# XiaoWang-Github/ORBIT-2

Measured on AMD Instinct MI355X. Metric: climate-grid samples/sec/node (fwd+bwd), interm_1b ERA5 1.4°→0.25°, 1/2/4/8 GPUs, higher is better.
Workload: dtype bf16

## Files before the change

orbit-2_amd/csrc/image.hip:

```cpp
#include "common.h"
#include "../../include/orbit2_hip.h"

namespace {

inline int grid_for(int64_t n, int per_block) {
  int64_t g = (n + per_block - 1) / per_block;
  if (g < 1) g = 1;
  if (g > 8192) g = 8192;
  return (int)g;
}

template <bool BWD, bool T_FP32 = false>
__global__ __launch_bounds__(256) void unpatchify_kernel(bf16_t* __restrict__ t, float* __restrict__ img, int B, int C,
                                                         int Hh, int Wh, int p) {
  const int64_t per = (int64_t)C * Hh * Wh;
  const int64_t n = (int64_t)B * per;
  const int wf = Wh / p;
  for (int64_t e = (int64_t)blockIdx.x * 256 + threadIdx.x; e < n; e += (int64_t)gridDim.x * 256) {
    const int b = (int)(e / per);
    int64_t r = e - (int64_t)b * per;
    if (!BWD) {
      const int c = (int)(r / ((int64_t)Hh * Wh));
      r -= (int64_t)c * Hh * Wh;
      const int y = (int)(r / Wh), x = (int)(r - (int64_t)y * Wh);
      const int hh = y / p, pp = y - hh * p, ww = x / p, qq = x - ww * p;
      const int64_t ti = ((((int64_t)hh * wf + ww) * p + pp) * p + qq) * C + c;
      img[e] = T_FP32 ? reinterpret_cast<const float*>(t)[(int64_t)b * per + ti] : bf2f(t[(int64_t)b * per + ti]);
    } else {
      const int c = (int)(r % C);
      int64_t q = r / C;
      const int qq = (int)(q % p); q /= p;
      const int pp = (int)(q % p); q /= p;
      const int ww = (int)(q % wf);
      const int hh = (int)(q / wf);
      t[e] = f2bf(img[(int64_t)b * per + ((int64_t)c * Hh + (hh * p + pp)) * Wh + (ww * p + qq)]);
    }
  }
}

constexpr int CONV_MAXCIN = 8;
constexpr int COB = 16;
__global__ __launch_bounds__(256) void conv3x3_fwd_kernel(const float* __restrict__ in, const int* __restrict__ cidx,
                                                          int in_ctotal, const float* __restrict__ wgt,
                                                          const float* __restrict__ bias, float* __restrict__ out,
                                                          float* __restrict__ pre, const float* __restrict__ addend,
                                                          int Ha, int Wa, int B, int Cin, int Cout, int H, int W,
                                                          int mode, int r) {
  __shared__ float sw[COB * CONV_MAXCIN * 9 + COB];
  const int co0 = blockIdx.y * COB;
  const int nco = (Cout - co0) < COB ? (Cout - co0) : COB;
  for (int e = threadIdx.x; e < nco * Cin * 9; e += 256) sw[e] = wgt[(size_t)co0 * Cin * 9 + e];
  for (int e = threadIdx.x; e < nco; e += 256) sw[COB * CONV_MAXCIN * 9 + e] = bias[co0 + e];
  __syncthreads();
  const int64_t npix = (int64_t)B * H * W;
  for (int64_t px = (int64_t)blockIdx.x * 256 + threadIdx.x; px < npix; px += (int64_t)gridDim.x * 256) {
    const int b = (int)(px / ((int64_t)H * W));
    const int rem = (int)(px - (int64_t)b * H * W);
    const int y = rem / W, x = rem - y * W;
    float nb[CONV_MAXCIN][9];
#pragma unroll
    for (int ci = 0; ci < CONV_MAXCIN; ++ci) {
      if (ci < Cin) {
        const int cs = cidx ? cidx[ci] : ci;
        const float* pl = in + ((size_t)b * in_ctotal + cs) * H * W;
#pragma unroll
        for (int k = 0; k < 9; ++k) {
          const int yy = y + k / 3 - 1, xx = x + k % 3 - 1;
          nb[ci][k] = (yy >= 0 && yy < H && xx >= 0 && xx < W) ? pl[(size_t)yy * W + xx] : 0.f;
        }
      }
    }
    for (int co = 0; co < nco; ++co) {
      float acc = sw[COB * CONV_MAXCIN * 9 + co];
#pragma unroll
      for (int ci = 0; ci < CONV_MAXCIN; ++ci) {
        if (ci < Cin) {
#pragma unroll
          for (int k = 0; k < 9; ++k) acc = fmaf(sw[(co * Cin + ci) * 9 + k], nb[ci][k], acc);
        }
      }
      const int cg = co0 + co;
      if (mode == 0) {
        if (addend) acc += addend[(((size_t)b * Cout + cg) * Ha + y) * Wa + x];
        out[(((size_t)b * Cout + cg) * H + y) * W + x] = acc;
      } else {
        pre[(((size_t)b * Cout + cg) * H + y) * W + x] = acc;
        const int rr = r * r;
        const int oc = cg / rr, sub = cg - oc * rr;
        out[(((size_t)b * (Cout / rr) + oc) * (H * r) + (y * r + sub / r)) * (size_t)(W * r) + (x * r + sub % r)] =
            gelu_f(acc);
      }
    }
  }
}

__device__ __forceinline__ float conv_dpre(const float* __restrict__ dout, const float* __restrict__ pre, int b,
                                           int co, int y, int x, int Cout, int H, int W, int mode, int r) {
  if (mode == 0) return dout[(((size_t)b * Cout + co) * H + y) * W + x];
  const int rr = r * r;
  const int oc = co / rr, sub = co - oc * rr;
  const float d =
      dout[(((size_t)b * (Cout / rr) + oc) * (H * r) + (y * r + sub / r)) * (size_t)(W * r) + (x * r + sub % r)];
  return d * dgelu_f(pre[(((size_t)b * Cout + co) * H + y) * W + x]);
}

__global__ __launch_bounds__(256) void conv3x3_bwd_data_kernel(const float* __restrict__ dout,
                                                               const float* __restrict__ pre,
                                                               const float* __restrict__ wgt, float* __restrict__ din,
                                                               int B, int Cin, int Cout, int H, int W, int mode,
                                                               int r) {
  const int64_t n = (int64_t)B * Cin * H * W;
  for (int64_t e = (int64_t)blockIdx.x * 256 + threadIdx.x; e < n; e += (int64_t)gridDim.x * 256) {
    int64_t q = e;
    const int x = (int)(q % W); q /= W;
    const int y = (int)(q % H); q /= H;
    const int ci = (int)(q % Cin);
    const int b = (int)(q / Cin);
    float acc = 0.f;
    for (int co = 0; co < Cout; ++co) {
#pragma unroll
      for (int k = 0; k < 9; ++k) {
        const int yy = y + 1 - k / 3, xx = x + 1 - k % 3;
        if (yy >= 0 && yy < H && xx >= 0 && xx < W)
          acc = fmaf(conv_dpre(dout, pre, b, co, yy, xx, Cout, H, W, mode, r), wgt[((size_t)co * Cin + ci) * 9 + k],
                     acc);
      }
    }
    din[e] = acc;
  }
}

constexpr int TW = 16, TH = 16;
__global__ __launch_bounds__(256) void conv3x3_bwd_weight_kernel(const float* __restrict__ dout,
                                                                 const float* __restrict__ pre,
                                                                 const float* __restrict__ in,
                                                                 const int* __restrict__ cidx, int in_ctotal,
                                                                 float* __restrict__ ws,
                                                                 int B, int Cin, int Cout, int H, int W, int mode,
                                                                 int r) {
  float* dw = ws + ((size_t)blockIdx.y * gridDim.x + blockIdx.x) * ((size_t)Cout * Cin * 9 + Cout);
  float* dbias = dw + (size_t)Cout * Cin * 9;
  __shared__ float sd[COB][TH][TW];
  __shared__ float si[CONV_MAXCIN][TH + 2][TW + 2];
  const int tiles_x = (W + TW - 1) / TW;
  const int ty0 = (blockIdx.x / tiles_x) * TH, tx0 = (blockIdx.x % tiles_x) * TW;
  const int b = blockIdx.y;
  for (int e = threadIdx.x; e < Cin * (TH + 2) * (TW + 2); e += 256) {
    const int ci = e / ((TH + 2) * (TW + 2));
    const int rem = e - ci * (TH + 2) * (TW + 2);
    const int yy = ty0 + rem / (TW + 2) - 1, xx = tx0 + rem % (TW + 2) - 1;
    const int cs = cidx ? cidx[ci] : ci;
    si[ci][rem / (TW + 2)][rem % (TW + 2)] =
        (yy >= 0 && yy < H && xx >= 0 && xx < W) ? in[(((size_t)b * in_ctotal + cs) * H + yy) * W + xx] : 0.f;
  }
  for (int co0 = 0; co0 < Cout; co0 += COB) {
    const int nco = (Cout - co0) < COB ? (Cout - co0) : COB;
    __syncthreads();
    for (int e = threadIdx.x; e < nco * TH * TW; e += 256) {
      const int co = e / (TH * TW);
      const int rem = e - co * TH * TW;
      const int y = ty0 + rem / TW, x = tx0 + rem % TW;
      sd[co][rem / TW][rem % TW] =
          (y < H && x < W) ? conv_dpre(dout, pre, b, co0 + co, y, x, Cout, H, W, mode, r) : 0.f;
    }
    __syncthreads();
    for (int e = threadIdx.x; e < nco * Cin * 9; e += 256) {
      const int co = e / (Cin * 9);
      const int rem = e - co * Cin * 9;
      const int ci = rem / 9, k = rem - ci * 9;
      const int ky = k / 3, kx = k - ky * 3;
      float s = 0.f;
      for (int y = 0; y < TH; ++y)
#pragma unroll
        for (int x = 0; x < TW; ++x) s = fmaf(sd[co][y][x], si[ci][y + ky][x + kx], s);
      dw[((size_t)(co0 + co) * Cin + ci) * 9 + k] = s;
    }
    for (int co = threadIdx.x; co < nco; co += 256) {
      float s = 0.f;
      for (int y = 0; y < TH; ++y)
        for (int x = 0; x < TW; ++x) s += sd[co][y][x];
      dbias[co0 + co] = s;
    }
  }
}

__global__ __launch_bounds__(256) void clamp_channel_kernel(float* __restrict__ img, const float* __restrict__ ref,
                                                            float* __restrict__ dimg, int B, int C, int HW,
                                                            int chan) {
  const int64_t n = (int64_t)B * HW;
  for (int64_t e = (int64_t)blockIdx.x * 256 + threadIdx.x; e < n; e += (int64_t)gridDim.x * 256) {
    const int b = (int)(e / HW);
    const size_t off = ((size_t)b * C + chan) * HW + (e - (int64_t)b * HW);
    if (dimg) { if (!(ref[off] > 0.f)) dimg[off] = 0.f; }
    else img[off] = fmaxf(img[off], 0.f);
  }
}

__device__ __forceinline__ float sgn(float v) { return (v > 0.f) ? 1.f : ((v < 0.f) ? -1.f : 0.f); }

__global__ __launch_bounds__(256) void loss_fwd_kernel(const float* __restrict__ pred, const float* __restrict__ tgt,
                                                       int Ht, int Wt, const float* __restrict__ latw,
                                                       const float* __restrict__ chanw, float* __restrict__ part,
                                                       float* __restrict__ part2, int C, int H, int W, int kind) {
  const int plane = blockIdx.y;
  const int c = plane % C, b = plane / C;
  const float* p = pred + (size_t)plane * H * W;
  const float* t = tgt + ((size_t)b * C + c) * Ht * Wt;
  const float cw = chanw ? chanw[c] : 1.f;
  float s = 0.f, s2 = 0.f;
  for (int e = blockIdx.x * 256 + threadIdx.x; e < H * W; e += gridDim.x * 256) {
    const int i = e / W, j = e - i * W;
    const float pv = p[e];
    const float tv0 = t[(size_t)i * Wt + j];
    const float d = pv - tv0;
    float err = d * d;
// ... 109 lines not shown
  const int64_t n = (int64_t)B * C * h * s * w * s;
  hipLaunchKernelGGL(unpatchify_kernel<false>, dim3(grid_for(n, 256)), dim3(256), 0, (hipStream_t)stream, (bf16_t*)t,
                     img, B, C, h * s, w * s, p);
  O2_CHECK_LAUNCH();
  return O2_OK;
}
extern "C" int orbit2_unpatchify_fwd_f32(const float* t, float* img, int B, int C, int h, int w, int p, int s,
                                         void* stream) {
  if (!t || !img || B <= 0 || C <= 0 || p <= 0 || s <= 0 || (h * s) % p || (w * s) % p) return O2_ERR_ARG;
  const int64_t n = (int64_t)B * C * h * s * w * s;
  hipLaunchKernelGGL((unpatchify_kernel<false, true>), dim3(grid_for(n, 256)), dim3(256), 0, (hipStream_t)stream,
                     (bf16_t*)t, img, B, C, h * s, w * s, p);
  O2_CHECK_LAUNCH();
  return O2_OK;
}
extern "C" int orbit2_unpatchify_bwd(const float* dimg, void* dt, int B, int C, int h, int w, int p, int s,
                                     void* stream) {
  if (!dimg || !dt || B <= 0 || C <= 0 || p <= 0 || s <= 0 || (h * s) % p || (w * s) % p) return O2_ERR_ARG;
  const int64_t n = (int64_t)B * C * h * s * w * s;
  hipLaunchKernelGGL(unpatchify_kernel<true>, dim3(grid_for(n, 256)), dim3(256), 0, (hipStream_t)stream, (bf16_t*)dt,
                     (float*)dimg, B, C, h * s, w * s, p);
  O2_CHECK_LAUNCH();
  return O2_OK;
}

extern "C" int orbit2_conv3x3_fwd(const float* in, const int* chan_idx, int in_ctotal, const float* weight,
                                  const float* bias, float* out, float* pre, const float* addend, int Ha, int Wa,
                                  int B, int Cin, int Cout, int H, int W, int mode, int r, void* stream) {
  if (!in || !weight || !bias || !out || B <= 0 || Cin <= 0 || Cin > CONV_MAXCIN || Cout <= 0 || H <= 0 || W <= 0)
    return O2_ERR_ARG;
  if (mode == 1 && (!pre || r <= 0 || Cout % (r * r))) return O2_ERR_ARG;
  if (mode != 0 && mode != 1) return O2_ERR_ARG;
  if (addend && (mode != 0 || Ha < H || Wa < W)) return O2_ERR_ARG;
  dim3 grid(grid_for((int64_t)B * H * W, 256), (Cout + COB - 1) / COB);
  hipLaunchKernelGGL(conv3x3_fwd_kernel, grid, dim3(256), 0, (hipStream_t)stream, in, chan_idx, in_ctotal, weight,
                     bias, out, pre, addend, Ha, Wa, B, Cin, Cout, H, W, mode, r);
  O2_CHECK_LAUNCH();
  return O2_OK;
}

extern "C" int64_t orbit2_conv3x3_bwd_ws_floats(int B, int Cin, int Cout, int H, int W) {
  if (B <= 0 || Cin <= 0 || Cout <= 0 || H <= 0 || W <= 0) return 0;
  return (int64_t)B * ((W + TW - 1) / TW) * ((H + TH - 1) / TH) * ((int64_t)Cout * Cin * 9 + Cout);
}

extern "C" int orbit2_conv3x3_bwd(const float* dout, const float* in, const int* chan_idx, int in_ctotal,
                                  const float* weight, const float* pre, float* din, float* dweight, float* dbias,
                                  int B, int Cin, int Cout, int H, int W, int mode, int r, float* ws, void* stream) {
  if (!dout || !in || !weight || !dweight || !dbias || !ws || B <= 0 || Cin <= 0 || Cin > CONV_MAXCIN || Cout <= 0)
    return O2_ERR_ARG;
  if (mode == 1 && (!pre || r <= 0 || Cout % (r * r))) return O2_ERR_ARG;
  if (mode != 0 && mode != 1) return O2_ERR_ARG;
  hipStream_t s = (hipStream_t)stream;
  if (din) {
    hipLaunchKernelGGL(conv3x3_bwd_data_kernel, dim3(grid_for((int64_t)B * Cin * H * W, 256)), dim3(256), 0, s, dout,
                       pre, weight, din, B, Cin, Cout, H, W, mode, r);
    O2_CHECK_LAUNCH();
  }
  dim3 grid(((W + TW - 1) / TW) * ((H + TH - 1) / TH), B);
  hipLaunchKernelGGL(conv3x3_bwd_weight_kernel, grid, dim3(256), 0, s, dout, pre, in, chan_idx, in_ctotal, ws,
                     B, Cin, Cout, H, W, mode, r);
  const int nparts = (int)(grid.x * grid.y);
  const int64_t nw = (int64_t)Cout * Cin * 9, slab = nw + Cout;
  o2_sum_parts(ws, nparts, slab, dweight, nw, 1.0f, 1, s);
  o2_sum_parts(ws + nw, nparts, slab, dbias, Cout, 1.0f, 1, s);
  O2_CHECK_LAUNCH();
  return O2_OK;
}

extern "C" int orbit2_clamp_channel(float* img, int B, int C, int HW, int chan, void* stream) {
  if (!img || B <= 0 || C <= 0 || HW <= 0 || chan < 0 || chan >= C) return O2_ERR_ARG;
  hipLaunchKernelGGL(clamp_channel_kernel, dim3(grid_for((int64_t)B * HW, 256)), dim3(256), 0, (hipStream_t)stream,
                     img, (const float*)nullptr, (float*)nullptr, B, C, HW, chan);
  O2_CHECK_LAUNCH();
  return O2_OK;
}
extern "C" int orbit2_clamp_channel_bwd(const float* img_clamped, float* dimg, int B, int C, int HW, int chan,
                                        void* stream) {
  if (!img_clamped || !dimg || B <= 0 || C <= 0 || HW <= 0 || chan < 0 || chan >= C) return O2_ERR_ARG;
  hipLaunchKernelGGL(clamp_channel_kernel, dim3(grid_for((int64_t)B * HW, 256)), dim3(256), 0, (hipStream_t)stream,
                     (float*)nullptr, img_clamped, dimg, B, C, HW, chan);
  O2_CHECK_LAUNCH();
  return O2_OK;
}

static const int LOSS_NBLK = 64;
extern "C" int orbit2_loss_fwd(const float* pred, const float* target, int Ht, int Wt, const float* lat_w,
                               const float* chan_w, float* out, float* ws, int B, int C, int H, int W, int kind,
                               void* stream) {
  if (!pred || !target || !out || !ws || B <= 0 || C <= 0 || H <= 0 || W <= 0 || Ht < H || Wt < W) return O2_ERR_ARG;
  if (kind < 0 || kind > 2) return O2_ERR_ARG;
  hipStream_t s = (hipStream_t)stream;
  float* ws2 = ws + (size_t)B * C * LOSS_NBLK;
  hipLaunchKernelGGL(loss_fwd_kernel, dim3(LOSS_NBLK, B * C), dim3(256), 0, s, pred, target, Ht, Wt, lat_w, chan_w, ws,
                     ws2, C, H, W, kind);
// ... 315 lines not shown
```

orbit-2_amd/csrc/varagg.hip:

```cpp
#include <stdlib.h>
#include "tiles32.h"
#include "../../include/orbit2_hip.h"

namespace {

constexpr int VA_T = 16;
constexpr int VA_MAXV = 32;
constexpr int VA_MAXH = 32;

template <int P>
__device__ __forceinline__ float va_row(const f32x4* g, const float* p, int j) {
  float val = g[0][j] * p[0];
#pragma unroll
  for (int c = 1; c < P * P; ++c) val += g[c][j] * p[c];
  return val + g[P * P][j];
}

constexpr int VA_LDS_LIMIT = 160 * 1024;

template <bool BWD, bool ZF32 = false, int P = 2>
__global__ __launch_bounds__(256) void varagg_kernel(const float* __restrict__ x, const float* __restrict__ stab,
                                                     const float* __restrict__ gtab, bf16_t* __restrict__ z,
                                                     float* __restrict__ attw, const bf16_t* __restrict__ dz,
                                                     float* __restrict__ dstab, float* __restrict__ dgtab, int B,
                                                     int V, int h, int w, int H, int D) {
  constexpr int PP = P * P, C = PP + 1;
  extern __shared__ __attribute__((aligned(16))) float sm[];
  float* pt = sm;
  float* aw = pt + VA_T * V * C;
  float* da = aw + VA_T * H * V;
  const int tid = threadIdx.x;
  const int Lw = w / P, L = (h / P) * Lw;
  const int64_t tok0 = (int64_t)blockIdx.x * VA_T;
  const int64_t ntok = (int64_t)B * L;
  const int dh = D / H;

  for (int e = tid; e < VA_T * V * C; e += 256) {
    const int c = e % C, v = (e / C) % V, t = e / (C * V);
    const int64_t tok = tok0 + t;
    float val = 0.f;
    if (tok < ntok) {
      if (c == PP) val = 1.f;
      else {
        const int b = (int)(tok / L), l = (int)(tok - (int64_t)b * L);
        const int pr = l / Lw, pc = l - pr * Lw;
        val = x[(((size_t)b * V + v) * h + (P * pr + c / P)) * w + P * pc + c % P];
      }
    }
    pt[e] = val;
  }
  __syncthreads();
  if (!BWD) {
    for (int e = tid; e < VA_T * H; e += 256) {
      const int hh = e % H, t = e / H;
      const float* st = stab + (size_t)hh * V * C;
      const float* pp = pt + (size_t)t * V * C;
      float mx = -1e30f;
      for (int v = 0; v < V; ++v) {
        float s = 0.f;
#pragma unroll
        for (int c = 0; c < C; ++c) s += st[v * C + c] * pp[v * C + c];
        mx = fmaxf(mx, s);
      }
      float sum = 0.f;
      for (int v = 0; v < V; ++v) {
        float s = 0.f;
#pragma unroll
        for (int c = 0; c < C; ++c) s += st[v * C + c] * pp[v * C + c];
        sum += __expf(s - mx);
      }
      const float inv = 1.f / sum;
      const int64_t tok = tok0 + t;
      for (int v = 0; v < V; ++v) {
        float s = 0.f;
#pragma unroll
        for (int c = 0; c < C; ++c) s += st[v * C + c] * pp[v * C + c];
        const float a = __expf(s - mx) * inv;
        aw[(t * H + hh) * V + v] = a;
        if (tok < ntok && (!ZF32 || attw)) attw[((size_t)tok * H + hh) * V + v] = a;
      }
    }
  } else {
    for (int e = tid; e < VA_T * H * V; e += 256) {
      const int64_t tok = tok0 + e / (H * V);
      aw[e] = tok < ntok ? attw[(size_t)tok0 * H * V + e] : 0.f;
      da[e] = 0.f;
    }
  }
  __syncthreads();
  const int nchunk = D / 4;
  for (int ch = tid; ch < nchunk; ch += 256) {
    const int i0 = ch * 4;
    const int hh = i0 / dh;
    if (!BWD) {
      float acc[VA_T][4];
#pragma unroll
      for (int t = 0; t < VA_T; ++t) { acc[t][0] = acc[t][1] = acc[t][2] = acc[t][3] = 0.f; }
      for (int v = 0; v < V; ++v) {
        f32x4 g[C];
#pragma unroll
        for (int c = 0; c < C; ++c) g[c] = *reinterpret_cast<const f32x4*>(gtab + ((size_t)(v * C + c)) * D + i0);
#pragma unroll
        for (int t = 0; t < VA_T; ++t) {
          const float* p = pt + (t * V + v) * C;
          const float a = aw[(t * H + hh) * V + v];
#pragma unroll
          for (int j = 0; j < 4; ++j) acc[t][j] += a * va_row<P>(g, p, j);
        }
      }
// ... 274 lines not shown
}

static int varagg_bwd_splits(int ntok, int H, int* cpw_out) {
  const int nchunk = (ntok + VM_T - 1) / VM_T;
  int splits = (768 + H - 1) / H;
  if (splits > nchunk) splits = nchunk;
  const int cpw = (nchunk + splits - 1) / splits;
  if (cpw_out) *cpw_out = cpw;
  return (nchunk + cpw - 1) / cpw;
}

template <int DH>
static void varagg_bwd_mfma_launch(const float* x, const float* gtab, const float* attw, const void* dz, float* dstab,
                                   float* dgtab, int B, int V, int h, int w, int H, int D, int ntok, float* ws, hipStream_t s) {
  int cpw;
  const int splits = varagg_bwd_splits(ntok, H, &cpw);
  float* ws_s = ws;
  float* ws_g = ws + (size_t)splits * H * V * 5;
  const size_t shm = (size_t)VM_T * DH * 2 + 2 * (size_t)VM_T * VM_NV * 2 +
                     sizeof(float) * (size_t)(VM_T * VM_GS + VM_T * V * 4 + 2 * VM_T * V);
  static bool attr_set = false;
  if (!attr_set) {
    (void)hipFuncSetAttribute((const void*)varagg_bwd_mfma_kernel<DH>, hipFuncAttributeMaxDynamicSharedMemorySize,
                              160 * 1024);
    attr_set = true;
  }
  hipLaunchKernelGGL(varagg_bwd_mfma_kernel<DH>, dim3((unsigned)H, (unsigned)splits), dim3(256), shm, s, x, gtab, attw,
                     (const bf16_t*)dz, ws_s, ws_g, B, V, h, w, H, D, cpw);
  o2_sum_parts(ws_s, splits, (int64_t)H * V * 5, dstab, (int64_t)H * V * 5, 1.0f, 1, s);
  o2_sum_parts(ws_g, splits, (int64_t)V * 5 * D, dgtab, (int64_t)V * 5 * D, 1.0f, 1, s);
}


constexpr int VT_T = 32;

template <int P>
__global__ __launch_bounds__(256) void varagg_ds_kernel(const float* __restrict__ x, const float* __restrict__ gtab,
                                                        const float* __restrict__ attw, const bf16_t* __restrict__ dz,
                                                        float* __restrict__ ds, int B, int V, int h, int w, int H, int D) {
  constexpr int PP = P * P, C = PP + 1;
  extern __shared__ __attribute__((aligned(16))) float sm[];
  float* pt = sm;
  float* aw = pt + VA_T * V * C;
  float* da = aw + VA_T * H * V;
  float* part = da + VA_T * H * V;
  const int tid = threadIdx.x;
  const int Lw = w / P, L = (h / P) * Lw;
  const int64_t tok0 = (int64_t)blockIdx.x * VA_T;
  const int64_t ntok = (int64_t)B * L;
  const int dh = D / H;
  const int gs = dh / 4;

  for (int e = tid; e < VA_T * V * C; e += 256) {
    const int c = e % C, v = (e / C) % V, t = e / (C * V);
    const int64_t tok = tok0 + t;
    float val = 0.f;
    if (tok < ntok) {
      if (c == PP) val = 1.f;
      else {
        const int b = (int)(tok / L), l = (int)(tok - (int64_t)b * L);
        const int pr = l / Lw, pc = l - pr * Lw;
        val = x[(((size_t)b * V + v) * h + (P * pr + c / P)) * w + P * pc + c % P];
      }
    }
    pt[e] = val;
  }
// ... 200 lines not shown
  int rpw;
  const int splits = varagg_tabgrad_splits(ntok, V, &rpw);
  float* ws_ds = ws;
  float* ws_s = ws_ds + (size_t)ntok * H * V;
  float* ws_g = ws_s + (size_t)splits * H * V * C;
  static bool attr_set = false;
  if (!attr_set) {
    (void)hipFuncSetAttribute((const void*)varagg_ds_kernel<P>, hipFuncAttributeMaxDynamicSharedMemorySize, VA_LDS_LIMIT);
    attr_set = true;
  }
  hipLaunchKernelGGL(varagg_ds_kernel<P>, dim3((unsigned)((ntok + VA_T - 1) / VA_T)), dim3(256), va_ds_lds(P, V, H), s, x, gtab,
                     attw, (const bf16_t*)dz, ws_ds, B, V, h, w, H, D);
  hipLaunchKernelGGL(varagg_tabgrad_kernel<P>, dim3((unsigned)V, (unsigned)splits), dim3(256), 0, s, x, attw, ws_ds,
                     (const bf16_t*)dz, ws_s, ws_g, B, V, h, w, H, D, rpw);
  o2_sum_parts(ws_s, splits, (int64_t)H * V * C, dstab, (int64_t)H * V * C, 1.0f, 1, s);
  o2_sum_parts(ws_g, splits, (int64_t)V * C * D, dgtab, (int64_t)V * C * D, 1.0f, 1, s);
}

}

static int va_check(int B, int V, int h, int w, int H, int D, int P = 2) {
  if (P != 1 && P != 2 && P != 4) return O2_ERR_ARG;
  if (B <= 0 || V <= 0 || V > VA_MAXV || H <= 0 || H > VA_MAXH || D <= 0 || h <= 0 || w <= 0) return O2_ERR_ARG;
  if ((h % P) || (w % P) || (D % 4) || (D % H) || ((D / H) % 4)) return O2_ERR_ARG;
  return O2_OK;
}

extern "C" int orbit2_varagg_fwd(const float* x, const float* stab, const float* gtab, void* z, float* attw, int B,
                                 int V, int h, int w, int H, int D, void* stream) {
  if (!x || !stab || !gtab || !z || !attw) return O2_ERR_ARG;
  int rc = va_check(B, V, h, w, H, D);
  if (rc) return rc;
  const int64_t ntok = (int64_t)B * (h / 2) * (w / 2);
  const size_t shm = sizeof(float) * (size_t)(VA_T * V * 5 + 2 * VA_T * H * V);
  hipLaunchKernelGGL(varagg_kernel<false>, dim3((unsigned)((ntok + VA_T - 1) / VA_T)), dim3(256), shm,
                     (hipStream_t)stream, x, stab, gtab, (bf16_t*)z, attw, (const bf16_t*)nullptr, (float*)nullptr,
                     (float*)nullptr, B, V, h, w, H, D);
  O2_CHECK_LAUNCH();
  return O2_OK;
}

extern "C" int orbit2_varagg_fwd_f32(const float* x, const float* stab, const float* gtab, float* z, float* attw, int B,
                                     int V, int h, int w, int H, int D, void* stream) {
  if (!x || !stab || !gtab || !z) return O2_ERR_ARG;
  int rc = va_check(B, V, h, w, H, D);
  if (rc) return rc;
  const int64_t ntok = (int64_t)B * (h / 2) * (w / 2);
  const size_t shm = sizeof(float) * (size_t)(VA_T * V * 5 + 2 * VA_T * H * V);
  hipLaunchKernelGGL((varagg_kernel<false, true>), dim3((unsigned)((ntok + VA_T - 1) / VA_T)), dim3(256), shm,
                     (hipStream_t)stream, x, stab, gtab, (bf16_t*)z, attw, (const bf16_t*)nullptr, (float*)nullptr,
                     (float*)nullptr, B, V, h, w, H, D);
  O2_CHECK_LAUNCH();
  return O2_OK;
}

extern "C" int64_t orbit2_varagg_bwd_ws_floats(int B, int V, int h, int w, int H, int D) {
  if (va_check(B, V, h, w, H, D)) return 0;
  const int64_t ntok = (int64_t)B * (h / 2) * (w / 2);
  if (ntok >= (1ll << 31) - 64) return 0;
  return (int64_t)varagg_bwd_splits((int)ntok, H, nullptr) * ((int64_t)H * V * 5 + (int64_t)V * 5 * D);
}

static bool varagg_bwd_fixed_order(int64_t ntok, int V, int H, int D) {
  static const bool force_scalar = getenv("ORBIT2_VARAGG_SCALAR") != nullptr;
  const int dh = D / H;
  return !force_scalar && (dh == 64 || dh == 128 || dh == 256) && 5 * V <= VM_NV && ntok < (1ll << 31) - 64;
// ... 142 lines not shown
```

Baseline: 18.02.

## Tile 3x3 convs through shared memory and add MFMA variable-aggregation forward

Rewrites the 3x3 conv forward, backward-data and backward-weight kernels. Each now stages a 16x64 input or gradient tile with halo into LDS, and each thread computes several output rows from register windows, with CIN as a template parameter. A vectorized pixel-shuffle store path is added for r=4. The backward-weight kernel becomes persistent and accumulates per-thread partial weight gradients across tiles. A bf16 hi/lo split MFMA kernel is also added for the variable-aggregation forward, meant to replace the scalar path for common head sizes. Together these target redundant global loads and scalar FMA cost, but raise register pressure and risk precision or coverage gaps for unsupported shapes.

New measurement: 18.12, median of 6. No clear change (+0.5%).

```diff
diff --git a/orbit-2_amd/csrc/image.hip b/orbit-2_amd/csrc/image.hip
--- a/orbit-2_amd/csrc/image.hip
+++ b/orbit-2_amd/csrc/image.hip
@@ -40,55 +40,123 @@
 
 constexpr int CONV_MAXCIN = 8;
 constexpr int COB = 16;
+constexpr int CT_H = 16, CT_W = 64;
+constexpr int CT_LW = CT_W + 4;
+constexpr int CT_RW = CT_H / 4;
+
+template <int U, class LoadF, class StoreF>
+__device__ __forceinline__ void conv_stage(int n, LoadF ld, StoreF st) {
+  for (int e0 = threadIdx.x; e0 < n; e0 += 256 * U) {
+    float v[U];
+#pragma unroll
+    for (int u = 0; u < U; ++u) v[u] = e0 + u * 256 < n ? ld(e0 + u * 256) : 0.f;
+#pragma unroll
+    for (int u = 0; u < U; ++u)
+      if (e0 + u * 256 < n) st(e0 + u * 256, v[u]);
+  }
+}
+
+template <int CIN, int U = 8>
+__device__ __forceinline__ void conv_stage_in(float (*si)[CT_H + 2][CT_LW], const float* __restrict__ in,
+                                              const int* __restrict__ cidx, int in_ctotal, int b, int ty0, int tx0, int H,
+                                              int W) {
+  constexpr int PL = (CT_H + 2) * (CT_W + 2);
+  conv_stage<U>(
+      CIN * PL,
+      [&](int e) {
+        const int ci = e / PL, rem = e - ci * PL;
+        const int ry = rem / (CT_W + 2), rx = rem - ry * (CT_W + 2);
+        const int yy = ty0 + ry - 1, xx = tx0 + rx - 1;
+        const int cs = cidx ? cidx[ci] : ci;
+        return (yy >= 0 && yy < H && xx >= 0 && xx < W) ? in[(((size_t)b * in_ctotal + cs) * H + yy) * W + xx] : 0.f;
+      },
+      [&](int e, float v) {
+        const int ci = e / PL, rem = e - ci * PL;
+        const int ry = rem / (CT_W + 2), rx = rem - ry * (CT_W + 2);
+        si[ci][ry][rx] = v;
+      });
+}
+
+template <int CIN, bool PS4>
 __global__ __launch_bounds__(256) void conv3x3_fwd_kernel(const float* __restrict__ in, const int* __restrict__ cidx,
                                                           int in_ctotal, const float* __restrict__ wgt,
                                                           const float* __restrict__ bias, float* __restrict__ out,
                                                           float* __restrict__ pre, const float* __restrict__ addend,
-                                                          int Ha, int Wa, int B, int Cin, int Cout, int H, int W,
-                                                          int mode, int r) {
-  __shared__ float sw[COB * CONV_MAXCIN * 9 + COB];
+                                                          int Ha, int Wa, int Cout, int H, int W, int mode, int r,
+                                                          int tiles_x, int tiles_y) {
+  __shared__ float si[CIN][CT_H + 2][CT_LW];
+  const int b = blockIdx.x / (tiles_x * tiles_y), trem = blockIdx.x - b * tiles_x * tiles_y;
+  const int ty0 = (trem / tiles_x) * CT_H, tx0 = (trem % tiles_x) * CT_W;
   const int co0 = blockIdx.y * COB;
   const int nco = (Cout - co0) < COB ? (Cout - co0) : COB;
-  for (int e = threadIdx.x; e < nco * Cin * 9; e += 256) sw[e] = wgt[(size_t)co0 * Cin * 9 + e];
-  for (int e = threadIdx.x; e < nco; e += 256) sw[COB * CONV_MAXCIN * 9 + e] = bias[co0 + e];
+  conv_stage_in<CIN>(si, in, cidx, in_ctotal, b, ty0, tx0, H, W);
   __syncthreads();
-  const int64_t npix = (int64_t)B * H * W;
-  for (int64_t px = (int64_t)blockIdx.x * 256 + threadIdx.x; px < npix; px += (int64_t)gridDim.x * 256) {
-    const int b = (int)(px / ((int64_t)H * W));
-    const int rem = (int)(px - (int64_t)b * H * W);
-    const int y = rem / W, x = rem - y * W;
-    float nb[CONV_MAXCIN][9];
-#pragma unroll
-    for (int ci = 0; ci < CONV_MAXCIN; ++ci) {
-      if (ci < Cin) {
-        const int cs = cidx ? cidx[ci] : ci;
-        const float* pl = in + ((size_t)b * in_ctotal + cs) * H * W;
-#pragma unroll
-        for (int k = 0; k < 9; ++k) {
-          const int yy = y + k / 3 - 1, xx = x + k % 3 - 1;
-          nb[ci][k] = (yy >= 0 && yy < H && xx >= 0 && xx < W) ? pl[(size_t)yy * W + xx] : 0.f;
+  const int lane = threadIdx.x & 63, yl0 = (threadIdx.x >> 6) * CT_RW;
+  const int x = tx0 + lane, y0 = ty0 + yl0;
+  if (x >= W || y0 >= H) return;
+  float nb[CIN][CT_RW + 2][3];
+#pragma unroll
+  for (int ci = 0; ci < CIN; ++ci)
+#pragma unroll
+    for (int i = 0; i < CT_RW + 2; ++i)
+#pragma unroll
+      for (int kx = 0; kx < 3; ++kx) nb[ci][i][kx] = si[ci][yl0 + i][lane + kx];
+  if (PS4) {
+    const int oc_n = Cout / 16;
+    for (int cg = 0; cg < nco; cg += 4) {
+      const int cgl = co0 + cg;
+      const int oc = cgl >> 4, sy = (cgl & 15) >> 2;
+      float acc[CT_RW][4];
+#pragma unroll
+      for (int j = 0; j < 4; ++j) {
+        const float* wc = wgt + (size_t)(cgl + j) * CIN * 9;
+        const float bs = bias[cgl + j];
+#pragma unroll
+        for (int rr = 0; rr < CT_RW; ++rr) {
+          float a = bs;
+#pragma unroll
+          for (int ci = 0; ci < CIN; ++ci)
+#pragma unroll
+            for (int k = 0; k < 9; ++k) a = fmaf(wc[ci * 9 + k], nb[ci][rr + k / 3][k % 3], a);
+          acc[rr][j] = a;
         }
       }
-    }
-    for (int co = 0; co < nco; ++co) {
-      float acc = sw[COB * CONV_MAXCIN * 9 + co];
-#pragma unroll
-      for (int ci = 0; ci < CONV_MAXCIN; ++ci) {
-        if (ci < Cin) {
-#pragma unroll
-          for (int k = 0; k < 9; ++k) acc = fmaf(sw[(co * Cin + ci) * 9 + k], nb[ci][k], acc);
+#pragma unroll
+      for (int rr = 0; rr < CT_RW; ++rr) {
+        const int y = y0 + rr;
+        if (y < H) {
+#pragma unroll
+          for (int j = 0; j < 4; ++j) pre[(((size_t)b * Cout + cgl + j) * H + y) * W + x] = acc[rr][j];
+          const f32x4 o = {gelu_f(acc[rr][0]), gelu_f(acc[rr][1]), gelu_f(acc[rr][2]), gelu_f(acc[rr][3])};
+          *reinterpret_cast<f32x4*>(out + (((size_t)b * oc_n + oc) * (H * 4) + (y * 4 + sy)) * (size_t)(W * 4) + x * 4) = o;
         }
       }
-      const int cg = co0 + co;
-      if (mode == 0) {
-        if (addend) acc += addend[(((size_t)b * Cout + cg) * Ha + y) * Wa + x];
-        out[(((size_t)b * Cout + cg) * H + y) * W + x] = acc;
-      } else {
-        pre[(((size_t)b * Cout + cg) * H + y) * W + x] = acc;
-        const int rr = r * r;
-        const int oc = cg / rr, sub = cg - oc * rr;
-        out[(((size_t)b * (Cout / rr) + oc) * (H * r) + (y * r + sub / r)) * (size_t)(W * r) + (x * r + sub % r)] =
-            gelu_f(acc);
+    }
+    return;
+  }
+  for (int co = 0; co < nco; ++co) {
+    const int cg = co0 + co;
+    const float* wc = wgt + (size_t)cg * CIN * 9;
+    const float bs = bias[cg];
+#pragma unroll
+    for (int rr = 0; rr < CT_RW; ++rr) {
+      const int y = y0 + rr;
+      float acc = bs;
+#pragma unroll
+      for (int ci = 0; ci < CIN; ++ci)
+#pragma unroll
+        for (int k = 0; k < 9; ++k) acc = fmaf(wc[ci * 9 + k], nb[ci][rr + k / 3][k % 3], acc);
+      if (y < H) {
+        if (mode == 0) {
+          if (addend) acc += addend[(((size_t)b * Cout + cg) * Ha + y) * Wa + x];
+          out[(((size_t)b * Cout + cg) * H + y) * W + x] = acc;
+        } else {
+          pre[(((size_t)b * Cout + cg) * H + y) * W + x] = acc;
+          const int rr2 = r * r;
+          const int oc = cg / rr2, sub = cg - oc * rr2;
+          out[(((size_t)b * (Cout / rr2) + oc) * (H * r) + (y * r + sub / r)) * (size_t)(W * r) + (x * r + sub % r)] =
+              gelu_f(acc);
+        }
       }
     }
   }
@@ -104,83 +172,212 @@
   return d * dgelu_f(pre[(((size_t)b * Cout + co) * H + y) * W + x]);
 }
 
+constexpr int DCB = 8;
+template <int CIN>
 __global__ __launch_bounds__(256) void conv3x3_bwd_data_kernel(const float* __restrict__ dout,
                                                                const float* __restrict__ pre,
                                                                const float* __restrict__ wgt, float* __restrict__ din,
-                                                               int B, int Cin, int Cout, int H, int W, int mode,
-                                                               int r) {
-  const int64_t n = (int64_t)B * Cin * H * W;
-  for (int64_t e = (int64_t)blockIdx.x * 256 + threadIdx.x; e < n; e += (int64_t)gridDim.x * 256) {
-    int64_t q = e;
-    const int x = (int)(q % W); q /= W;
-    const int y = (int)(q % H); q /= H;
-    const int ci = (int)(q % Cin);
-    const int b = (int)(q / Cin);
-    float acc = 0.f;
-    for (int co = 0; co < Cout; ++co) {
-#pragma unroll
-      for (int k = 0; k < 9; ++k) {
-        const int yy = y + 1 - k / 3, xx = x + 1 - k % 3;
-        if (yy >= 0 && yy < H && xx >= 0 && xx < W)
-          acc = fmaf(conv_dpre(dout, pre, b, co, yy, xx, Cout, H, W, mode, r), wgt[((size_t)co * Cin + ci) * 9 + k],
-                     acc);
-      }
-    }
-    din[e] = acc;
-  }
-}
-
-constexpr int TW = 16, TH = 16;
-__global__ __launch_bounds__(256) void conv3x3_bwd_weight_kernel(const float* __restrict__ dout,
+                                                               int Cout, int H, int W, int mode, int r, int tiles_x,
+                                                               int tiles_y) {
+  __shared__ float sd[DCB][CT_H + 2][CT_LW];
+  constexpr int PL = (CT_H + 2) * (CT_W + 2);
+  const int b = blockIdx.x / (tiles_x * tiles_y), trem = blockIdx.x - b * tiles_x * tiles_y;
+  const int ty0 = (trem / tiles_x) * CT_H, tx0 = (trem % tiles_x) * CT_W;
+  const int lane = threadIdx.x & 63, yl0 = (threadIdx.x >> 6) * CT_RW;
+  const int rs = (mode == 1 && DCB % r == 0) ? r : 1;
+  float acc[CIN][CT_RW];
+#pragma unroll
+  for (int ci = 0; ci < CIN; ++ci)
+#pragma unroll
+    for (int rr = 0; rr < CT_RW; ++rr) acc[ci][rr] = 0.f;
+  for (int co0 = 0; co0 < Cout; co0 += DCB) {
+    const int nco = (Cout - co0) < DCB ? (Cout - co0) : DCB;
+    if (co0) __syncthreads();
+    conv_stage<8>(
+        nco * PL,
+        [&](int e) {
+          const int sx = e % rs, q = e / rs;
+          const int rx = q % (CT_W + 2), q2 = q / (CT_W + 2);
+          const int ry = q2 % (CT_H + 2), cl = (q2 / (CT_H + 2)) * rs + sx;
+          const int yy = ty0 + ry - 1, xx = tx0 + rx - 1;
+          return (yy >= 0 && yy < H && xx >= 0 && xx < W) ? conv_dpre(dout, pre, b, co0 + cl, yy, xx, Cout, H, W, mode, r)
+                                                         : 0.f;
+        },
+        [&](int e, float v) {
+          const int sx = e % rs, q = e / rs;
+          const int rx = q % (CT_W + 2), q2 = q / (CT_W + 2);
+          const int ry = q2 % (CT_H + 2), cl = (q2 / (CT_H + 2)) * rs + sx;
+          sd[cl][ry][rx] = v;
+        });
+    __syncthreads();
+    for (int cl = 0; cl < nco; ++cl) {
+      float nbd[CT_RW + 2][3];
+#pragma unroll
+      for (int i = 0; i < CT_RW + 2; ++i)
+#pragma unroll
+        for (int j = 0; j < 3; ++j) nbd[i][j] = sd[cl][yl0 + i][lane + j];
+      const float* wc = wgt + (size_t)(co0 + cl) * CIN * 9;
+#pragma unroll
+      for (int ci = 0; ci < CIN; ++ci)
+#pragma unroll
+        for (int k = 0; k < 9; ++k)
+#pragma unroll
+          for (int rr = 0; rr < CT_RW; ++rr) acc[ci][rr] = fmaf(nbd[rr + 2 - k / 3][2 - k % 3], wc[ci * 9 + k], acc[ci][rr]);
+    }
+  }
+  const int x = tx0 + lane;
+  if (x >= W) return;
+#pragma unroll
+  for (int ci = 0; ci < CIN; ++ci)
+#pragma unroll
+    for (int rr = 0; rr < CT_RW; ++rr) {
+      const int y = ty0 + yl0 + rr;
+      if (y < H) din[(((size_t)b * CIN + ci) * H + y) * W + x] = acc[ci][rr];
+    }
+}
+
+template <int CIN> struct ConvWG {
+  static constexpr int FIT = 100 / (CIN * 9);
+  static constexpr int NCO = FIT < 1 ? 1 : (FIT > 4 ? 4 : FIT);
+  static constexpr int NE = CIN * 9 + 1;
+  static constexpr int RG = NCO == 1 ? 16 : (NCO == 2 ? 8 : 4);
+  static constexpr int SU = NCO == 1 ? 16 : 8;
+};
+static int conv_wg_nco(int Cin) {
+  const int fit = 100 / (Cin * 9);
+  return fit < 1 ? 1 : (fit > 4 ? 4 : fit);
+}
+static int conv_wg_plan(int B, int Cin, int Cout, int H, int W, int* wco_out, int* gy_out) {
+  const int nco = conv_wg_nco(Cin);
+  int wco = 1;
+  while (wco < 4 && wco * nco < Cout) wco *= 2;
+  const int gy = (Cout + wco * nco - 1) / (wco * nco);
+  const int64_t ntiles = (int64_t)B * ((W + CT_W - 1) / CT_W) * ((H + CT_H - 1) / CT_H);
+  int64_t g = 512 / gy;
+  if (g < 1) g = 1;
+  if (g > ntiles) g = ntiles;
+  if (wco_out) *wco_out = wco;
+  if (gy_out) *gy_out = gy;
+  return (int)g;
+}
+
+template <int CIN>
+__global__ __launch_bounds__(256, 2) void conv3x3_bwd_weight_kernel(const float* __restrict__ dout,
                                                                  const float* __restrict__ pre,
                                                                  const float* __restrict__ in,
                                                                  const int* __restrict__ cidx, int in_ctotal,
-                                                                 float* __restrict__ ws,
-                                                                 int B, int Cin, int Cout, int H, int W, int mode,
-                                                                 int r) {
-  float* dw = ws + ((size_t)blockIdx.y * gridDim.x + blockIdx.x) * ((size_t)Cout * Cin * 9 + Cout);
-  float* dbias = dw + (size_t)Cout * Cin * 9;
-  __shared__ float sd[COB][TH][TW];
-  __shared__ float si[CONV_MAXCIN][TH + 2][TW + 2];
-  const int tiles_x = (W + TW - 1) / TW;
-  const int ty0 = (blockIdx.x / tiles_x) * TH, tx0 = (blockIdx.x % tiles_x) * TW;
-  const int b = blockIdx.y;
-  for (int e = threadIdx.x; e < Cin * (TH + 2) * (TW + 2); e += 256) {
-    const int ci = e / ((TH + 2) * (TW + 2));
-    const int rem = e - ci * (TH + 2) * (TW + 2);
-    const int yy = ty0 + rem / (TW + 2) - 1, xx = tx0 + rem % (TW + 2) - 1;
-    const int cs = cidx ? cidx[ci] : ci;
-    si[ci][rem / (TW + 2)][rem % (TW + 2)] =
-        (yy >= 0 && yy < H && xx >= 0 && xx < W) ? in[(((size_t)b * in_ctotal + cs) * H + yy) * W + xx] : 0.f;
-  }
-  for (int co0 = 0; co0 < Cout; co0 += COB) {
-    const int nco = (Cout - co0) < COB ? (Cout - co0) : COB;
+                                                                 float* __restrict__ ws, int B, int Cout, int H, int W,
+                                                                 int mode, int r, int wco) {
+  constexpr int NCO = ConvWG<CIN>::NCO, NE = ConvWG<CIN>::NE, RG = ConvWG<CIN>::RG;
+  __shared__ float si[CIN][CT_H + 2][CT_LW];
+  __shared__ float red[4][NCO * NE];
+  const int lane = threadIdx.x & 63, wave = threadIdx.x >> 6;
+  const int wr = 4 / wco;
+  const int wc = wave % wco, wrow = wave / wco;
+  const int rows = CT_H / wr;
+  const int cob = (blockIdx.y * wco + wc) * NCO;
+  const int tiles_x = (W + CT_W - 1) / CT_W, tiles_y = (H + CT_H - 1) / CT_H;
+  const int ntiles = B * tiles_x * tiles_y;
+  float acc[NCO][CIN][9], bacc[NCO];
+#pragma unroll
+  for (int j = 0; j < NCO; ++j) {
+    bacc[j] = 0.f;
+#pragma unroll
+    for (int ci = 0; ci < CIN; ++ci)
+#pragma unroll
+      for (int k = 0; k < 9; ++k) acc[j][ci][k] = 0.f;
+  }
+  for (int tile = blockIdx.x; tile < ntiles; tile += gridDim.x) {
+    const int b = tile / (tiles_x * tiles_y), trem = tile - b * tiles_x * tiles_y;
+    const int ty0 = (trem / tiles_x) * CT_H, tx0 = (trem % tiles_x) * CT_W;
+    const int x = tx0 + lane, yl0 = wrow * rows;
+    auto load_d = [&](float (&dd)[RG][NCO], int yl, int nr) {
+#pragma unroll
+      for (int rr = 0; rr < RG; ++rr)
+#pragma unroll
+        for (int j = 0; j < NCO; ++j) {
+          const int y = ty0 + yl + rr;
+          dd[rr][j] = (rr < nr && y < H && x < W && cob + j < Cout) ? conv_dpre(dout, pre, b, cob + j, y, x, Cout, H, W, mode, r)
+                                                                 : 0.f;
+        }
+    };
+    float d[RG][NCO];
+    load_d(d, yl0, rows);
     __syncthreads();
-    for (int e = threadIdx.x; e < nco * TH * TW; e += 256) {
-      const int co = e / (TH * TW);
-      const int rem = e - co * TH * TW;
-      const int y = ty0 + rem / TW, x = tx0 + rem % TW;
-      sd[co][rem / TW][rem % TW] =
-          (y < H && x < W) ? conv_dpre(dout, pre, b, co0 + co, y, x, Cout, H, W, mode, r) : 0.f;
-    }
+    conv_stage_in<CIN, ConvWG<CIN>::SU>(si, in, cidx, in_ctotal, b, ty0, tx0, H, W);
     __syncthreads();
-    for (int e = threadIdx.x; e < nco * Cin * 9; e += 256) {
-      const int co = e / (Cin * 9);
-      const int rem = e - co * Cin * 9;
-      const int ci = rem / 9, k = rem - ci * 9;
-      const int ky = k / 3, kx = k - ky * 3;
+    for (int g0 = 0; g0 < rows; g0 += RG) {
+      const int yl = yl0 + g0, nr = rows - g0;
+      float dn[RG][NCO];
+      load_d(dn, yl + RG, nr - RG);
+      float win[3][CIN][3];
+#pragma unroll
+      for (int i = 0; i < 2; ++i)
+#pragma unroll
+        for (int ci = 0; ci < CIN; ++ci)
+#pragma unroll
+          for (int kx = 0; kx < 3; ++kx) win[i][ci][kx] = si[ci][yl + i][lane + kx];
+#pragma unroll
+      for (int rr = 0; rr < RG; ++rr) {
+        if (rr < nr) {
+#pragma unroll
+          for (int ci = 0; ci < CIN; ++ci)
+#pragma unroll
+            for (int kx = 0; kx < 3; ++kx) win[(rr + 2) % 3][ci][kx] = si[ci][yl + rr + 2][lane + kx];
+#pragma unroll
+          for (int j = 0; j < NCO; ++j) {
+            bacc[j] += d[rr][j];
+#pragma unroll
+            for (int ci = 0; ci < CIN; ++ci)
+#pragma unroll
+              for (int k = 0; k < 9; ++k) acc[j][ci][k] = fmaf(d[rr][j], win[(rr + k / 3) % 3][ci][k % 3], acc[j][ci][k]);
+          }
+        }
+      }
+#pragma unroll
+      for (int rr = 0; rr < RG; ++rr)
+#pragma unroll
+        for (int j = 0; j < NCO; ++j) d[rr][j] = dn[rr][j];
+    }
+  }
+#pragma unroll
+  for (int j = 0; j < NCO; ++j) {
+#pragma unroll
+    for (int ci = 0; ci < CIN; ++ci)
+#pragma unroll
+      for (int k = 0; k < 9; ++k) {
+        const float s = wave_sum(acc[j][ci][k]);
+        if (lane == 0) red[wave][j * NE + ci * 9 + k] = s;
+      }
+    const float sb = wave_sum(bacc[j]);
+    if (lane == 0) red[wave][j * NE + CIN * 9] = sb;
+  }
+  __syncthreads();
+  float* dw = ws + (size_t)blockIdx.x * ((size_t)Cout * CIN * 9 + Cout);
+  float* dbias = dw + (size_t)Cout * CIN * 9;
+  for (int e = threadIdx.x; e < wco * NCO * NE; e += 256) {
+    const int wci = e / (NCO * NE), q = e - wci * (NCO * NE);
+    const int j = q / NE, i = q - j * NE;
+    const int co = (blockIdx.y * wco + wci) * NCO + j;
+    if (co < Cout) {
       float s = 0.f;
-      for (int y = 0; y < TH; ++y)
-#pragma unroll
-        for (int x = 0; x < TW; ++x) s = fmaf(sd[co][y][x], si[ci][y + ky][x + kx], s);
-      dw[((size_t)(co0 + co) * Cin + ci) * 9 + k] = s;
-    }
-    for (int co = threadIdx.x; co < nco; co += 256) {
-      float s = 0.f;
-      for (int y = 0; y < TH; ++y)
-        for (int x = 0; x < TW; ++x) s += sd[co][y][x];
-      dbias[co0 + co] = s;
-    }
+      for (int g = 0; g < wr; ++g) s += red[g * wco + wci][q];
+      if (i < CIN * 9) dw[(size_t)co * CIN * 9 + i] = s;
+      else dbias[co] = s;
+    }
+  }
+}
+
+template <class F> static inline void conv_with_cin(int Cin, F&& f) {
+  switch (Cin) {
+    case 1: f(o2_int<1>{}); break;
+    case 2: f(o2_int<2>{}); break;
+    case 3: f(o2_int<3>{}); break;
+    case 4: f(o2_int<4>{}); break;
+    case 5: f(o2_int<5>{}); break;
+    case 6: f(o2_int<6>{}); break;
+    case 7: f(o2_int<7>{}); break;
+    default: f(o2_int<8>{}); break;
   }
 }
 
@@ -356,35 +553,49 @@
   if (mode == 1 && (!pre || r <= 0 || Cout % (r * r))) return O2_ERR_ARG;
   if (mode != 0 && mode != 1) return O2_ERR_ARG;
   if (addend && (mode != 0 || Ha < H || Wa < W)) return O2_ERR_ARG;
-  dim3 grid(grid_for((int64_t)B * H * W, 256), (Cout + COB - 1) / COB);
-  hipLaunchKernelGGL(conv3x3_fwd_kernel, grid, dim3(256), 0, (hipStream_t)stream, in, chan_idx, in_ctotal, weight,
-                     bias, out, pre, addend, Ha, Wa, B, Cin, Cout, H, W, mode, r);
+  const int tiles_x = (W + CT_W - 1) / CT_W, tiles_y = (H + CT_H - 1) / CT_H;
+  if ((int64_t)B * tiles_x * tiles_y >= (1ll << 31)) return O2_ERR_ARG;
+  dim3 grid((unsigned)(B * tiles_x * tiles_y), (Cout + COB - 1) / COB);
+  const bool ps4 = mode == 1 && r == 4 && !((uintptr_t)out & 15);
+  conv_with_cin(Cin, [&](auto cin) {
+    constexpr int CIN = decltype(cin)::value;
+    if (ps4)
+      hipLaunchKernelGGL((conv3x3_fwd_kernel<CIN, true>), grid, dim3(256), 0, (hipStream_t)stream, in, chan_idx, in_ctotal,
+                         weight, bias, out, pre, addend, Ha, Wa, Cout, H, W, mode, r, tiles_x, tiles_y);
+    else
+      hipLaunchKernelGGL((conv3x3_fwd_kernel<CIN, false>), grid, dim3(256), 0, (hipStream_t)stream, in, chan_idx, in_ctotal,
+                         weight, bias, out, pre, addend, Ha, Wa, Cout, H, W, mode, r, tiles_x, tiles_y);
+  });
   O2_CHECK_LAUNCH();
   return O2_OK;
 }
 
 extern "C" int64_t orbit2_conv3x3_bwd_ws_floats(int B, int Cin, int Cout, int H, int W) {
-  if (B <= 0 || Cin <= 0 || Cout <= 0 || H <= 0 || W <= 0) return 0;
-  return (int64_t)B * ((W + TW - 1) / TW) * ((H + TH - 1) / TH) * ((int64_t)Cout * Cin * 9 + Cout);
+  if (B <= 0 || Cin <= 0 || Cin > CONV_MAXCIN || Cout <= 0 || H <= 0 || W <= 0) return 0;
+  return (int64_t)conv_wg_plan(B, Cin, Cout, H, W, nullptr, nullptr) * ((int64_t)Cout * Cin * 9 + Cout);
 }
 
 extern "C" int orbit2_conv3x3_bwd(const float* dout, const float* in, const int* chan_idx, int in_ctotal,
                                   const float* weight, const float* pre, float* din, float* dweight, float* dbias,
                                   int B, int Cin, int Cout, int H, int W, int mode, int r, float* ws, void* stream) {
-  if (!dout || !in || !weight || !dweight || !dbias || !ws || B <= 0 || Cin <= 0 || Cin > CONV_MAXCIN || Cout <= 0)
+  if (!dout || !in || !weight || !dweight || !dbias || !ws || B <= 0 || Cin <= 0 || Cin > CONV_MAXCIN || Cout <= 0 ||
+      H <= 0 || W <= 0)
     return O2_ERR_ARG;
   if (mode == 1 && (!pre || r <= 0 || Cout % (r * r))) return O2_ERR_ARG;
   if (mode != 0 && mode != 1) return O2_ERR_ARG;
+  const int tiles_x = (W + CT_W - 1) / CT_W, tiles_y = (H + CT_H - 1) / CT_H;
+  if ((int64_t)B * tiles_x * tiles_y >= (1ll << 31)) return O2_ERR_ARG;
   hipStream_t s = (hipStream_t)stream;
-  if (din) {
-    hipLaunchKernelGGL(conv3x3_bwd_data_kernel, dim3(grid_for((int64_t)B * Cin * H * W, 256)), dim3(256), 0, s, dout,
-                       pre, weight, din, B, Cin, Cout, H, W, mode, r);
-    O2_CHECK_LAUNCH();
-  }
-  dim3 grid(((W + TW - 1) / TW) * ((H + TH - 1) / TH), B);
-  hipLaunchKernelGGL(conv3x3_bwd_weight_kernel, grid, dim3(256), 0, s, dout, pre, in, chan_idx, in_ctotal, ws,
-                     B, Cin, Cout, H, W, mode, r);
-  const int nparts = (int)(grid.x * grid.y);
+  int wco, gy;
+  const int nparts = conv_wg_plan(B, Cin, Cout, H, W, &wco, &gy);
+  conv_with_cin(Cin, [&](auto cin) {
+    constexpr int CIN = decltype(cin)::value;
+    if (din)
+      hipLaunchKernelGGL(conv3x3_bwd_data_kernel<CIN>, dim3((unsigned)(B * tiles_x * tiles_y)), dim3(256), 0, s, dout, pre,
+                         weight, din, Cout, H, W, mode, r, tiles_x, tiles_y);
+    hipLaunchKernelGGL(conv3x3_bwd_weight_kernel<CIN>, dim3((unsigned)nparts, (unsigned)gy), dim3(256), 0, s, dout, pre, in,
+                       chan_idx, in_ctotal, ws, B, Cout, H, W, mode, r, wco);
+  });
   const int64_t nw = (int64_t)Cout * Cin * 9, slab = nw + Cout;
   o2_sum_parts(ws, nparts, slab, dweight, nw, 1.0f, 1, s);
   o2_sum_parts(ws + nw, nparts, slab, dbias, Cout, 1.0f, 1, s);
diff --git a/orbit-2_amd/csrc/varagg.hip b/orbit-2_amd/csrc/varagg.hip
--- a/orbit-2_amd/csrc/varagg.hip
+++ b/orbit-2_amd/csrc/varagg.hip
@@ -1,4 +1,5 @@
 #include <stdlib.h>
+#include <string.h>
 #include "tiles32.h"
 #include "../../include/orbit2_hip.h"
 
@@ -14,6 +15,14 @@
 #pragma unroll
   for (int c = 1; c < P * P; ++c) val += g[c][j] * p[c];
   return val + g[P * P][j];
+}
+
+template <int C>
+__device__ __forceinline__ float va_score(const float* st, const float* pp) {
+  float s = 0.f;
+#pragma unroll
+  for (int c = 0; c < C; ++c) s = fmaf(st[c], pp[c], s);
+  return s;
 }
 
 constexpr int VA_LDS_LIMIT = 160 * 1024;
@@ -57,24 +66,18 @@
       const float* pp = pt + (size_t)t * V * C;
       float mx = -1e30f;
       for (int v = 0; v < V; ++v) {
-        float s = 0.f;
-#pragma unroll
-        for (int c = 0; c < C; ++c) s += st[v * C + c] * pp[v * C + c];
+        const float s = va_score<C>(st + v * C, pp + v * C);
         mx = fmaxf(mx, s);
       }
       float sum = 0.f;
       for (int v = 0; v < V; ++v) {
-        float s = 0.f;
-#pragma unroll
-        for (int c = 0; c < C; ++c) s += st[v * C + c] * pp[v * C + c];
+        const float s = va_score<C>(st + v * C, pp + v * C);
         sum += __expf(s - mx);
       }
       const float inv = 1.f / sum;
       const int64_t tok = tok0 + t;
       for (int v = 0; v < V; ++v) {
-        float s = 0.f;
-#pragma unroll
-        for (int c = 0; c < C; ++c) s += st[v * C + c] * pp[v * C + c];
+        const float s = va_score<C>(st + v * C, pp + v * C);
         const float a = __expf(s - mx) * inv;
         aw[(t * H + hh) * V + v] = a;
         if (tok < ntok && (!ZF32 || attw)) attw[((size_t)tok * H + hh) * V + v] = a;
@@ -415,6 +418,215 @@
 }
 
 
+template <int DH> struct VF {
+  static constexpr int NTB = DH == 64 ? 2 : 1;
+  static constexpr int T = 32 * NTB;
+  static constexpr int DBW = (DH / 32) * NTB / 4;
+  static constexpr int ZRS = DH * 2 + 16;
+  static constexpr int NKS = VM_NV / 16;
+};
+
+template <int DH>
+__global__ __launch_bounds__(256, (DH == 256 ? 1 : 2)) void varagg_fwd_mfma_kernel(const float* __restrict__ x,
+                                                                 const float* __restrict__ stab,
+                                                                 const float* __restrict__ gtab, bf16_t* __restrict__ z,
+                                                                 float* __restrict__ attw, int B, int V, int h, int w, int H,
+                                                                 int D, int chunks_per_wg) {
+  using F = VF<DH>;
+  using CA = Cfg<VM_NV>;
+  constexpr int T = F::T, NTB = F::NTB, DBW = F::DBW, NKS = F::NKS;
+  __shared__ __attribute__((aligned(16))) char a2hi[T * CA::RB];
+  __shared__ __attribute__((aligned(16))) char a2lo[T * CA::RB];
+  __shared__ __attribute__((aligned(16))) float ev[T][VA_MAXV];
+  __shared__ __attribute__((aligned(16))) char zt[T * F::ZRS];
+  const int tid = threadIdx.x, lane = tid & 63;
+  const int wave = __builtin_amdgcn_readfirstlane(tid >> 6);
+  const int hq = lane >> 5;
+  const int hh = blockIdx.x;
+  const int Lw = w / 2, L = (h / 2) * Lw;
+  const int ntok = B * L;
+  const int nchunk = (ntok + T - 1) / T;
+  const int c0 = blockIdx.y * chunks_per_wg;
+  const int c1 = min(nchunk, c0 + chunks_per_wg);
+  if (c0 >= c1) return;
+  const int NV5 = 5 * V;
+  const int nks = (NV5 + 15) / 16;
+  const int tb = wave % NTB, db0 = (wave / NTB) * DBW;
+
+  bf16x8 gfh[DBW][NKS], gfl[DBW][NKS];
+#pragma unroll
+  for (int i = 0; i < DBW; ++i) {
+    const float* src = gtab + (size_t)hh * DH + (db0 + i) * 32 + (lane & 31);
+#pragma unroll
+    for (int ks = 0; ks < NKS; ++ks) {
+#pragma unroll
+      for (int j = 0; j < 8; ++j) {
+        const int row = ks * 16 + 8 * hq + j;
+        const float g = src[(size_t)min(row, NV5 - 1) * D];
+        bf16_t hi, lo;
+        split_bf16(row < NV5 ? g : 0.f, hi, lo);
+        gfh[i][ks][j] = (short)hi; gfl[i][ks][j] = (short)lo;
+      }
+    }
+  }
+  for (int e = tid; e < T * CA::RB / 16; e += 256) {
+    bf16x8 zz;
+#pragma unroll
+    for (int j = 0; j < 8; ++j) zz[j] = 0;
+    reinterpret_cast<bf16x8*>(a2hi)[e] = zz;
+    reinterpret_cast<bf16x8*>(a2lo)[e] = zz;
+  }
+  const int tl = tid >> 3, sub = tid & 7;
+  float st[4][5];
+#pragma unroll
+  for (int k = 0; k < 4; ++k) {
+    const int v = sub + 8 * k;
+#pragma unroll
+    for (int c = 0; c < 5; ++c) st[k][c] = v < V ? stab[((size_t)hh * V + v) * 5 + c] : 0.f;
+  }
+  float pn[NTB][4][4];
+  auto fetch = [&](int ch) {
+#pragma unroll
+    for (int tt = 0; tt < NTB; ++tt) {
+      const int tk = min(ch * T + tt * 32 + tl, ntok - 1);
+      const int b = tk / L, l = tk - b * L;
+      const int pr = l / Lw, pc = l - pr * Lw;
+      const float* xp = x + ((size_t)b * V * h + 2 * pr) * w + 2 * pc;
+#pragma unroll
+      for (int k = 0; k < 4; ++k) {
+        const int v = sub + 8 * k;
+        if (v < V) {
+          const o2_f32x2 r0 = *reinterpret_cast<const o2_f32x2*>(xp + (size_t)v * h * w);
+          const o2_f32x2 r1 = *reinterpret_cast<const o2_f32x2*>(xp + (size_t)v * h * w + w);
+          pn[tt][k][0] = r0[0]; pn[tt][k][1] = r0[1]; pn[tt][k][2] = r1[0]; pn[tt][k][3] = r1[1];
+        } else { pn[tt][k][0] = pn[tt][k][1] = pn[tt][k][2] = pn[tt][k][3] = 0.f; }
+      }
+    }
+  };
+  fetch(c0);
+  auto store_z = [&](int tok0) {
+    for (int e = tid; e < T * (DH / 8); e += 256) {
+      const int t = e / (DH / 8), cc = e - t * (DH / 8);
+      const int tok = tok0 + t;
+      if (tok < ntok)
+        *reinterpret_cast<u32x4*>(z + (size_t)tok * D + (size_t)hh * DH + cc * 8) =
+            *reinterpret_cast<const u32x4*>(zt + t * F::ZRS + cc * 16);
+    }
+  };
+
+  for (int ch = c0; ch < c1; ++ch) {
+    const int tok0 = ch * T;
+    float p[NTB][4][4], ex[NTB][4];
+#pragma unroll
+    for (int tt = 0; tt < NTB; ++tt)
+#pragma unroll
+      for (int k = 0; k < 4; ++k)
+#pragma unroll
+        for (int c = 0; c < 4; ++c) p[tt][k][c] = pn[tt][k][c];
+    if (ch + 1 < c1) fetch(ch + 1);
+#pragma unroll
+    for (int tt = 0; tt < NTB; ++tt) {
+      float s[4], mx = -1e30f;
+#pragma unroll
+      for (int k = 0; k < 4; ++k) {
+        const float p5[5] = {p[tt][k][0], p[tt][k][1], p[tt][k][2], p[tt][k][3], 1.f};
+        s[k] = va_score<5>(st[k], p5);
+        if (sub + 8 * k < V) mx = fmaxf(mx, s[k]);
+      }
+      mx = fmaxf(mx, __shfl_xor(mx, 1));
+      mx = fmaxf(mx, __shfl_xor(mx, 2));
+      mx = fmaxf(mx, __shfl_xor(mx, 4));
+#pragma unroll
+      for (int k = 0; k < 4; ++k) {
+        ex[tt][k] = __expf(s[k] - mx);
+        if (sub + 8 * k < V) ev[tt * 32 + tl][sub + 8 * k] = ex[tt][k];
+      }
+    }
+    __syncthreads();
+    if (ch > c0) store_z(tok0 - T);
+#pragma unroll
+    for (int tt = 0; tt < NTB; ++tt) {
+      const int t = tt * 32 + tl;
+      float sum = 0.f;
+      for (int v = 0; v < V; ++v) sum += ev[t][v];
+      const float inv = 1.f / sum;
+      const int tok = tok0 + t;
+#pragma unroll
+      for (int k = 0; k < 4; ++k) {
+        const int v = sub + 8 * k;
+        if (v < V) {
+          const float a = ex[tt][k] * inv;
+          if (tok < ntok) attw[((size_t)tok * H + hh) * V + v] = a;
+#pragma unroll
+          for (int c = 0; c < 5; ++c) {
+            const int col = 5 * v + c;
+            bf16_t hi, lo;
+            split_bf16(c < 4 ? a * p[tt][k][c] : a, hi, lo);
+            const int off = t * CA::RB + (((col >> 3) ^ swz<VM_NV>(t)) << 4) + (col & 7) * 2;
+            *reinterpret_cast<bf16_t*>(a2hi + off) = hi;
+            *reinterpret_cast<bf16_t*>(a2lo + off) = lo;
+          }
+        }
+      }
+    }
+    __syncthreads();
+    {
+      f32x16 acc[DBW];
+#pragma unroll
+      for (int i = 0; i < DBW; ++i)
+#pragma unroll
+        for (int r = 0; r < 16; ++r) acc[i][r] = 0.f;
+#pragma unroll
+      for (int ks = 0; ks < NKS; ++ks) {
+        if (ks < nks) {
+          const bf16x8 ah = row_frag<VM_NV>(a2hi, tb * 32 + (lane & 31), ks, hq);
+          const bf16x8 al = row_frag<VM_NV>(a2lo, tb * 32 + (lane & 31), ks, hq);
+#pragma unroll
+          for (int i = 0; i < DBW; ++i) {
+            acc[i] = MFMA32(gfl[i][ks], ah, acc[i]);
+            acc[i] = MFMA32(gfh[i][ks], al, acc[i]);
+            acc[i] = MFMA32(gfh[i][ks], ah, acc[i]);
+          }
+        }
+      }
+      char* zrow = zt + (tb * 32 + (lane & 31)) * F::ZRS;
+#pragma unroll
+      for (int i = 0; i < DBW; ++i)
+#pragma unroll
+        for (int g = 0; g < 4; ++g) {
+          u32x2 o;
+          o[0] = pack_bf2(acc[i][4 * g], acc[i][4 * g + 1]);
+          o[1] = pack_bf2(acc[i][4 * g + 2], acc[i][4 * g + 3]);
+          *reinterpret_cast<u32x2*>(zrow + ((db0 + i) * 32 + 8 * g + 4 * hq) * 2) = o;
+        }
+    }
+  }
+  __syncthreads();
+  store_z((c1 - 1) * T);
+}
+
+static bool varagg_fwd_on_mfma(int64_t ntok, int V, int H, int D) {
+  static const bool force_scalar = [] {
+    const char* e = getenv("ORBIT2_VARAGG_FWD");
+    return e && !strcmp(e, "scalar");
+  }();
+  const int dh = D / H;
+  return !force_scalar && (dh == 64 || dh == 128 || dh == 256) && 5 * V <= VM_NV && ntok < (1ll << 31) - 64;
+}
+
+template <int DH>
+static void varagg_fwd_mfma_launch(const float* x, const float* stab, const float* gtab, void* z, float* attw, int B, int V,
+                                   int h, int w, int H, int D, int ntok, hipStream_t s) {
+  const int nchunk = (ntok + VF<DH>::T - 1) / VF<DH>::T;
+  int splits = 512 / H < 1 ? 1 : 512 / H;
+  if (splits > nchunk) splits = nchunk;
+  const int cpw = (nchunk + splits - 1) / splits;
+  splits = (nchunk + cpw - 1) / cpw;
+  hipLaunchKernelGGL(varagg_fwd_mfma_kernel<DH>, dim3((unsigned)H, (unsigned)splits), dim3(256), 0, s, x, stab, gtab,
+                     (bf16_t*)z, attw, B, V, h, w, H, D, cpw);
+}
+
+
 constexpr int VT_T = 32;
 
 template <int P>
@@ -681,6 +893,15 @@
   int rc = va_check(B, V, h, w, H, D);
   if (rc) return rc;
   const int64_t ntok = (int64_t)B * (h / 2) * (w / 2);
+  if (varagg_fwd_on_mfma(ntok, V, H, D) && !((uintptr_t)x & 7)) {
+    hipStream_t s = (hipStream_t)stream;
+    const int dh = D / H;
+    if (dh == 64) varagg_fwd_mfma_launch<64>(x, stab, gtab, z, attw, B, V, h, w, H, D, (int)ntok, s);
+    else if (dh == 128) varagg_fwd_mfma_launch<128>(x, stab, gtab, z, attw, B, V, h, w, H, D, (int)ntok, s);
+    else varagg_fwd_mfma_launch<256>(x, stab, gtab, z, attw, B, V, h, w, H, D, (int)ntok, s);
+    O2_CHECK_LAUNCH();
+    return O2_OK;
+  }
   const size_t shm = sizeof(float) * (size_t)(VA_T * V * 5 + 2 * VA_T * H * V);
   hipLaunchKernelGGL(varagg_kernel<false>, dim3((unsigned)((ntok + VA_T - 1) / VA_T)), dim3(256), shm,
                      (hipStream_t)stream, x, stab, gtab, (bf16_t*)z, attw, (const bf16_t*)nullptr, (float*)nullptr,
```
